# JiehongLin/SAM-6D

Measured on NVIDIA H100. Metric: poses/sec, higher is better.
Workload: dtype bf16

## Files before the change

include/sam6d_b200.h:

```cpp
#ifndef SAM6D_B200_H
#define SAM6D_B200_H

#ifdef __cplusplus
extern "C" {
#endif


int sam6d_fps(const float* xyz, int b, int n, int m, float* temp, int* idx, void* stream);
int sam6d_fps_single_cta(const float* xyz, int b, int n, int m, float* temp, int* idx, void* stream);

int sam6d_gather_points(const float* points, const int* idx, int b, int c, int n, int m, float* out, void* stream);

int sam6d_gather_rows(const float* src, const int* idx, int b, int n, int m, int c, long long src_bstride, float* out,
                      void* stream);
int sam6d_gather_rows_bf16_f32(const void* src, const int* idx, int b, int n, int m, int c, long long src_bstride, float* out,
                               void* stream);

int sam6d_ball_query(const float* new_xyz, const float* xyz, int b, int n, int m, float radius, int nsample, int* idx,
                     int* cnt, void* stream);
int sam6d_ball_query_pair(const float* new_xyz, const float* xyz, int b, int n, int m, float radius_a, int nsample_a,
                          float radius_b, int nsample_b, int* idx_a, int* idx_b, int* cnt_a, int* cnt_b, void* stream);

int sam6d_group_points(const float* points, const int* idx, int b, int c, int n, int np, int ns, float* out, void* stream);

// ... 132 lines not shown
int sam6d_linattn_apply(const float* Qf, long long q_rpb, long long q_bs, long long q_ld, const float* KV, const float* KS,
                        int B, int H, float* X, long long x_bs, long long x_ld, void* stream);
int sam6d_linattn_kv_pack(const float* Kf, long long k_ld, long long k_bs, const float* V, long long v_ld, long long v_bs, int B,
                          int J, void* blob, float* KS, void* stream);
int sam6d_linattn_tc(const void* Q, long long q_ld, long long q_bs, const void* blob, const float* KS,
                     const float* softplus_scale, int B, int rpb, void* X, long long x_ld, long long x_bs, void* stream);

int sam6d_coarse_assign(const float* A, int B, int S, float* W, float* w1, void* stream);
int sam6d_coarse_sample(const float* W, int B, int L, const float* rand, int nr, int* idx, void* stream);
int sam6d_coarse_hypotheses(const int* idx, const float* pts1, const float* pts2, int B, int n, int n1, float* Rt,
                            float* resid, void* stream);
int sam6d_topk_smallest(const float* v, int B, int n, int k, int* out, void* stream);
int sam6d_coarse_select(const float* Rt, const int* top, int B, int n1, int n2, const float* pts1, const float* w1, int n,
                        const float* model, int nm, float* scores, float* R, float* t, void* stream);
int sam6d_coarse_pick_distinct(const float* Rt, const int* top, const float* scores, int B, int n1, int n2, int K, float cos_thr,
                               float d2_min, float* R_out, float* t_out, float* score_out, unsigned char* valid, int* count,
                               void* stream);
int sam6d_coarse_pick_distinct_sym(const float* Rt, const int* top, const float* scores, int B, int n1, int n2, int K, float cos_thr,
                                   float d2_min, const float* symR, const float* symt, int S, const int* sym_range, int max_count,
                                   const float* radius, float* R_out, float* t_out, float* score_out, unsigned char* valid,
                                   int* count, void* stream);


int sam6d_pe_mlp_max(const float* pts, const int* idx, const int* cnt, int B, int N, int ns, const float* W1,
                     const float* B1, const float* W2, const float* B2, const float* W3, const float* B3, float* out,
                     int out_ld, int out_off, void* stream);
int sam6d_pe_mlp_max_tc(const float* pts, const int* idx, int B, int N, int ns, const float* W1, const float* B1,
                        const void* W2_bf16, const float* B2, const void* W3_bf16, const float* B3, void* out, int out_is_bf16,
                        int out_ld, int out_off, void* stream);
int sam6d_fine_assign(const float* A, int B, int S, int ld, float shift, const float* pts2, float* rsum, float* csum, float* cpart,
                      int* cpi, int* lab1, int* lab2, float* wts, float* pred, void* stream);
int sam6d_fine_pass_tc(const void* Fa, const void* Fb, int B, int S, float alpha, float shift, int mode, const float* row_f,
                       const float* col_f, int ld_f, const float* q4, float* out_inv, int* lab, float* wts, float* pred, void* stream);
int sam6d_fine_masked_points(const int* lab2, const float* pts2, int B, int S, int ld, float* q4, void* stream);
int sam6d_weighted_procrustes(const float* src, const float* ref, const float* wts, int B, int N, float weight_thresh,
                              float eps, float* R, float* t, void* stream);
int sam6d_pose_score(const float* pts1, const int* lab1, int B, int N, const float* R, const float* t, const float* model,
                     int nm, float dis_thres, const float* radius, float* score, float* t_scaled, void* stream);

int sam6d_bilinear_gather(const void* up, int up_is_bf16, const long long* choose, int B, int K, int G, int sub, int C, int H, int W,
                          float* out, void* stream);

int sam6d_attn_relpos(const float* qkv, long long tok_ld, int nW, int Hs, int Ws, int nH, int head_dim, const float* rel_h,
                      const float* rel_w, float scale, void* out, int out_is_bf16, long long out_ld, void* stream);

int sam6d_attn_global_tc(const void* qkv, long long ld, const void* Vt, long long vt_ld, const void* rel_blob, int B, int H, int grid,
                         float scale, void* out, int out_is_bf16, long long out_ld, void* stream);
int sam6d_attn_global_tc_ex(const void* qkv, long long ld, const void* Vt, long long vt_ld, const void* rel_blob, int B, int H, int grid,
                            int head_dim, float scale, void* out, int out_is_bf16, long long out_ld, void* stream);

int sam6d_icp_refine(const float* R, const float* t, const float* pts, int B, int N, const float* samples, const float* normals,
                     int O, int M, const int* obj, const float* radius, int iters, float* R_out, float* t_out, int* inliers,
                     float* rms, int* iters_run, int* corr, double* sums, void* stream);
int sam6d_icp_max_samples(void);

int sam6d_track_points(const float* rdepth, const unsigned short* depth, int O, int H, int W, float depth_scale, float fx, float fy,
                       float cx, float cy, const float* centre, const float* radius, int margin, int N, unsigned char* hmask,
                       unsigned char* cand, int* rows, float* pts, int* count, int* index, void* stream);
int sam6d_track_points_scene(const float* rdepth, const unsigned short* depth, int L, int H, int W, float depth_scale, float fx,
                             float fy, float cx, float cy, const float* centre, const float* radius, int margin, int N,
                             unsigned char* hmask, unsigned char* dmask, unsigned char* cand, int* rows, float* pts, int* count,
                             int* index, void* stream);

int sam6d_pose_verify(const float* rdepth, const float* depth, const unsigned char* mask, const int* mrow, const float* tau, int P,
                      int M, int H, int W, float rscale, int* counts, void* stream);

// ... 50 lines not shown
```

sam6d_b200/_lib.py:

```python
import ctypes
import os
import re

import torch

_Tensor = torch.Tensor

_HERE = os.path.dirname(os.path.abspath(__file__))
HEADER = os.path.join(os.path.dirname(_HERE), "include", "sam6d_b200.h")
LIB_PATH = os.path.join(_HERE, "libsam6d_b200.so")

_CTYPES = {
    "int": ctypes.c_int,
    "long long": ctypes.c_longlong,
    "float": ctypes.c_float,
    "double": ctypes.c_double,
}


def parse_header(path: str = HEADER):
    text = open(path).read()
    text = re.sub(r"/\*.*?\*/", "", text, flags=re.S)
    protos = {}
    for m in re.finditer(r"(const char\*|int)\s+(sam6d_\w+)\s*\(([^)]*)\)\s*;", text):
# ... 8 lines not shown
                typ, nm = a.rsplit(" ", 1)
                argl.append((_CTYPES[typ.strip()], nm))
        protos[name] = (ctypes.c_char_p if ret != "int" else ctypes.c_int, argl)
    return protos


class Sam6dError(RuntimeError):
    pass


_lib = None
_protos = None
_fns = {}


def lib():
    global _lib, _protos
    if _lib is None:
        if not os.path.exists(LIB_PATH):
            raise Sam6dError(
                f"{LIB_PATH} not found: build it with `python -m sam6d_b200.build` "
                "(or __graft_entry__.build()); sam6d_b200 has no CPU or eager fallback")
        _lib = ctypes.CDLL(LIB_PATH)
        _protos = parse_header()
        for name, (ret, args) in _protos.items():
            fn = getattr(_lib, name)
            fn.restype = ret
            fn.argtypes = [t for t, _ in args]
            _fns[name] = (fn, len(args) - 1 if args and args[-1][1] == "stream" else -1)
    return _lib


_launches = 0
_MULTI = {"sam6d_fine_assign": 6, "sam6d_coarse_select": 2, "sam6d_geo_embed_tc": 2, "sam6d_render_meshes": 4, "sam6d_yolo_masks": 2,
          "sam6d_mask_rle_count": 2, "sam6d_template_score_agg": 2, "sam6d_template_score": 2,
          "sam6d_pbr_reference_crops": 2, "sam6d_track_points": 4,
          "sam6d_track_points_scene": 5, "sam6d_symmetry_agreement": 2}
_timed = {}


def launch_count() -> int:
    return _launches


def add_launches(n: int):
    global _launches
    _launches += int(n)


def time_kernel(name: str, enable: bool = True):
    if enable:
        _timed[name] = []
    else:
        _timed.pop(name, None)


def timed_events(name: str):
    return _timed.get(name, [])


def call(name: str, *args):
    global _launches
    if _lib is None:
        lib()
    fn, n_before_stream = _fns[name]
    args = [(a.data_ptr() if a.is_cuda else _not_device(name, a)) if isinstance(a, _Tensor) else a for a in args]
    if len(args) == n_before_stream:
# ... 25 lines not shown
```

sam6d_b200/csrc/coarse.cu:

```cuda
#include "common.cuh"
#include "svd3.cuh"

namespace {

constexpr int ASSIGN_THREADS = 1024;
__global__ void __launch_bounds__(ASSIGN_THREADS) coarse_assign_kernel(const float* __restrict__ A, int S, float* __restrict__ W,
                                                            float* __restrict__ w1out) {
  extern __shared__ float sm[];
  float* a = sm;
  float* rmax = a + S * S;
  float* rsum = rmax + S;
  float* cmax = rsum + S;
  float* csum = cmax + S;
  int* lab1 = (int*)(csum + S);
  int* lab2 = lab1 + S;
  const int b = blockIdx.x, tid = threadIdx.x, lane = tid & 31, warp = tid >> 5;
  const float* Ab = A + (size_t)b * S * S;
  for (int e = tid; e < S * S; e += ASSIGN_THREADS) a[e] = Ab[e];
  __syncthreads();
  for (int i = warp; i < S; i += ASSIGN_THREADS / 32) {
    float m = -INFINITY;
    for (int j = lane; j < S; j += 32) m = fmaxf(m, a[i * S + j]);
    m = warp_max(m);
    float s = 0.f;
// ... 11 lines not shown
  __syncthreads();
  for (int e = tid; e < S * S; e += ASSIGN_THREADS) {
    int i = e / S, j = e - i * S;
    float v = a[e];
    a[e] = (expf(v - rmax[i]) / rsum[i]) * (expf(v - cmax[j]) / csum[j]);
  }
  __syncthreads();
  for (int i = warp; i < S; i += ASSIGN_THREADS / 32) {
    float bv = -INFINITY; int bi = 0x7fffffff;
    for (int j = lane; j < S; j += 32) argmax_first(bv, bi, a[i * S + j], j);
    warp_argmax_first(bv, bi);
    if (lane == 0) lab1[i] = bi;
  }
  for (int j = tid; j < S; j += ASSIGN_THREADS) {
    float bv = -INFINITY; int bi = 0;
    for (int i = 0; i < S; ++i) { float v = a[i * S + j]; if (v > bv) { bv = v; bi = i; } }
    lab2[j] = bi;
  }
  __syncthreads();
  const int n = S - 1;
  float* Wb = W + (size_t)b * n * n;
  for (int e = tid; e < n * n; e += ASSIGN_THREADS) {
    int i = e / n, j = e - i * n;
    float v = a[(i + 1) * S + (j + 1)];
    v = v * (lab1[i + 1] > 0 ? 1.f : 0.f) * (lab2[j + 1] > 0 ? 1.f : 0.f);
    Wb[e] = v * sqrtf(v);
  }
  for (int i = tid; i < n; i += ASSIGN_THREADS) w1out[(size_t)b * n + i] = lab1[i + 1] > 0 ? 1.f : 0.f;
}

__global__ void __launch_bounds__(1024) coarse_sample_kernel(const float* __restrict__ W, int L, const float* __restrict__ rand,
                                                             int nr, int* __restrict__ idx_out) {
  extern __shared__ float cdf[];
  __shared__ double part[1024];
  const int b = blockIdx.x, tid = threadIdx.x;
  const float* Wb = W + (size_t)b * L;
  const int per = (L + 1023) / 1024;
  const int beg = min(tid * per, L), end = min(beg + per, L);
  double s = 0.0;
  for (int i = beg; i < end; ++i) s += (double)Wb[i];
  part[tid] = s;
  __syncthreads();
  for (int o = 1; o < 1024; o <<= 1) {
    double v = (tid >= o) ? part[tid - o] : 0.0;
    __syncthreads();
    part[tid] += v;
    __syncthreads();
  }
  double run = (tid == 0) ? 0.0 : part[tid - 1];
  for (int i = beg; i < end; ++i) { run += (double)Wb[i]; cdf[i] = (float)run; }
  __syncthreads();
  const float denom = cdf[L - 1] + 1e-8f;
  __syncthreads();
  for (int i = tid; i < L; i += 1024) cdf[i] = cdf[i] / denom;
  __syncthreads();
  for (int r = tid; r < nr; r += 1024) {
    float v = rand[(size_t)b * nr + r];
    int lo = 0, hi = L;
    while (lo < hi) {
      int mid = (lo + hi) >> 1;
      if (cdf[mid] < v) lo = mid + 1; else hi = mid;
    }
    idx_out[(size_t)b * nr + r] = lo;
  }
}

__global__ void __launch_bounds__(128) coarse_hyp_kernel(const int* __restrict__ idx, const float* __restrict__ pts1,
                                                         const float* __restrict__ pts2, int n, int n1, float* __restrict__ Rt,
                                                         float* __restrict__ resid) {
  const int b = blockIdx.y;
  const int hpt = blockIdx.x * blockDim.x + threadIdx.x;
  if (hpt >= n1) return;
  const int* id = idx + ((size_t)b * n1 + hpt) * 3;
  float p1[3][3], p2[3][3];
  int i1s[3], i2s[3];
#pragma unroll
  for (int k = 0; k < 3; ++k) {
    int v = id[k];
    int i1 = min(v / n, n - 1), i2 = min(v % n, n - 1);
    i1s[k] = i1; i2s[k] = i2;
    const float* a = pts1 + ((size_t)b * n + i1) * 3;
    const float* c = pts2 + ((size_t)b * n + i2) * 3;
#pragma unroll
// ... 24 lines not shown
  if (rank0) {
#pragma unroll
    for (int i = 0; i < 3; ++i)
#pragma unroll
      for (int j = 0; j < 3; ++j) Rd[i][j] = (i == j) ? 1.0 : 0.0;
  } else {
    procrustes_rotation(H, Rd, rank1);
  }
  float R[3][3], t[3];
#pragma unroll
  for (int i = 0; i < 3; ++i)
#pragma unroll
    for (int j = 0; j < 3; ++j) R[i][j] = (float)Rd[i][j];
#pragma unroll
  for (int i = 0; i < 3; ++i) t[i] = cr[i] - (R[i][0] * cs[0] + R[i][1] * cs[1] + R[i][2] * cs[2]);
  float rs = 0.f;
#pragma unroll
  for (int k = 0; k < 3; ++k) {
    float x = p1[k][0] - t[0], y = p1[k][1] - t[1], z = p1[k][2] - t[2];
    float ex = x * R[0][0] + y * R[1][0] + z * R[2][0] - p2[k][0];
    float ey = x * R[0][1] + y * R[1][1] + z * R[2][1] - p2[k][1];
    float ez = x * R[0][2] + y * R[1][2] + z * R[2][2] - p2[k][2];
    rs += sqrtf(ex * ex + ey * ey + ez * ez);
  }
  float* o = Rt + ((size_t)b * n1 + hpt) * 12;
#pragma unroll
  for (int i = 0; i < 3; ++i)
#pragma unroll
    for (int j = 0; j < 3; ++j) o[i * 3 + j] = R[i][j];
  o[9] = t[0]; o[10] = t[1]; o[11] = t[2];
  resid[(size_t)b * n1 + hpt] = rs / 3.f;
}

__global__ void __launch_bounds__(1024) topk_smallest_kernel(const float* __restrict__ v, int n, int npow2, int k,
                                                             int* __restrict__ out) {
  extern __shared__ unsigned long long keys[];
  const int b = blockIdx.x, tid = threadIdx.x;
  for (int i = tid; i < npow2; i += 1024) {
    unsigned long long key = ~0ull;
    if (i < n) {
      float f = v[(size_t)b * n + i];
      unsigned u = __float_as_uint(f);
      u = (u & 0x80000000u) ? ~u : (u | 0x80000000u);
      key = ((unsigned long long)u << 32) | (unsigned)i;
    }
    keys[i] = key;
  }
  __syncthreads();
  for (int size = 2; size <= npow2; size <<= 1) {
    for (int stride = size >> 1; stride > 0; stride >>= 1) {
      for (int i = tid; i < npow2 / 2; i += 1024) {
        int lo = 2 * i - (i & (stride - 1));
        int hi = lo + stride;
        bool asc = ((lo & size) == 0);
        unsigned long long a = keys[lo], c = keys[hi];
        if ((a > c) == asc) { keys[lo] = c; keys[hi] = a; }
      }
      __syncthreads();
    }
  }
  for (int i = tid; i < k; i += 1024) out[(size_t)b * k + i] = (int)(keys[i] & 0xffffffffu);
}

constexpr int SEL_PP = 4, SEL_THREADS = 224;
__device__ __forceinline__ float min3f(float a, float b, float c) { return fminf(fminf(a, b), c); }
__global__ void __launch_bounds__(SEL_THREADS) coarse_select_kernel(const float* __restrict__ Rt, const int* __restrict__ top, int n1,
                                                                    int n2, const float* __restrict__ pts1, const float* __restrict__ w1,
                                                                    int n, const float* __restrict__ model, int nm,
                                                                    float* __restrict__ scores) {
  extern __shared__ float4 smq[];
  __shared__ float red[2 * SEL_PP][SEL_THREADS / 32];
  __shared__ float rts[SEL_PP][12];
  const int pose0 = blockIdx.x * SEL_PP, b = blockIdx.y, tid = threadIdx.x;
  for (int i = tid; i < nm; i += SEL_THREADS) {
    const float* q = model + ((size_t)b * nm + i) * 3;
    const float x = q[0], y = q[1], z = q[2];
    smq[i] = make_float4(x, y, z, x * x + y * y + z * z);
  }
  if (tid < SEL_PP * 12) {
    const int pp = tid / 12, e = tid - pp * 12;
    const int pose = min(pose0 + pp, n2 - 1);
    rts[pp][e] = Rt[((size_t)b * n1 + top[(size_t)b * n2 + pose]) * 12 + e];
  }
  __syncthreads();
  float num = 0.f, den[SEL_PP];
#pragma unroll
  for (int pp = 0; pp < SEL_PP; ++pp) den[pp] = 0.f;
  for (int i = tid; i < n; i += SEL_THREADS) {
    const float* p = pts1 + ((size_t)b * n + i) * 3;
    const float px = p[0], py = p[1], pz = p[2];
    float ax[SEL_PP], ay[SEL_PP], az[SEL_PP], x2[SEL_PP], best[SEL_PP];
#pragma unroll
    for (int pp = 0; pp < SEL_PP; ++pp) {
      const float* R = rts[pp];
// ... 209 lines not shown
  if (B == 0) return 0;
  size_t smem = ((size_t)S * S + 6 * S) * sizeof(float);
  S6_REQUIRE(smem <= 220 * 1024);
  S6_CHECK(cudaFuncSetAttribute(coarse_assign_kernel, cudaFuncAttributeMaxDynamicSharedMemorySize, (int)smem));
  coarse_assign_kernel<<<B, ASSIGN_THREADS, smem, s6_stream(stream)>>>(A, S, W, w1);
  S6_LAUNCH_CHECK();
  return 0;
}

S6_API int sam6d_coarse_sample(const float* W, int B, int L, const float* rand, int nr, int* idx, void* stream) {
  S6_REQUIRE(W && rand && idx && B >= 0 && L > 0 && nr >= 0);
  if (B == 0 || nr == 0) return 0;
  size_t smem = (size_t)L * sizeof(float);
  S6_REQUIRE(smem <= 200 * 1024);
  S6_CHECK(cudaFuncSetAttribute(coarse_sample_kernel, cudaFuncAttributeMaxDynamicSharedMemorySize, (int)smem));
  coarse_sample_kernel<<<B, 1024, smem, s6_stream(stream)>>>(W, L, rand, nr, idx);
  S6_LAUNCH_CHECK();
  return 0;
}

S6_API int sam6d_coarse_hypotheses(const int* idx, const float* pts1, const float* pts2, int B, int n, int n1, float* Rt,
                                   float* resid, void* stream) {
  S6_REQUIRE(idx && pts1 && pts2 && Rt && resid && B >= 0 && n > 0 && n1 >= 0);
  if (B == 0 || n1 == 0) return 0;
  dim3 grid(s6_cdiv(n1, 128), B);
  coarse_hyp_kernel<<<grid, 128, 0, s6_stream(stream)>>>(idx, pts1, pts2, n, n1, Rt, resid);
  S6_LAUNCH_CHECK();
  return 0;
}

S6_API int sam6d_topk_smallest(const float* v, int B, int n, int k, int* out, void* stream) {
  S6_REQUIRE(v && out && B >= 0 && n > 0 && k > 0 && k <= n);
  if (B == 0) return 0;
  int npow2 = 2;
  while (npow2 < n) npow2 <<= 1;
  size_t smem = (size_t)npow2 * sizeof(unsigned long long);
  S6_REQUIRE(smem <= 200 * 1024);
  S6_CHECK(cudaFuncSetAttribute(topk_smallest_kernel, cudaFuncAttributeMaxDynamicSharedMemorySize, (int)smem));
  topk_smallest_kernel<<<B, 1024, smem, s6_stream(stream)>>>(v, n, npow2, k, out);
  S6_LAUNCH_CHECK();
  return 0;
}

S6_API int sam6d_coarse_select(const float* Rt, const int* top, int B, int n1, int n2, const float* pts1, const float* w1, int n,
                               const float* model, int nm, float* scores, float* R, float* t, void* stream) {
  S6_REQUIRE(Rt && top && pts1 && w1 && model && scores && R && t && B >= 0 && n > 0 && nm > 0 && n2 > 0);
  if (B == 0) return 0;
  size_t smem = (size_t)nm * 4 * sizeof(float);
  S6_REQUIRE(smem <= 200 * 1024);
  S6_CHECK(cudaFuncSetAttribute(coarse_select_kernel, cudaFuncAttributeMaxDynamicSharedMemorySize, (int)smem));
  dim3 grid(s6_cdiv(n2, SEL_PP), B);
  coarse_select_kernel<<<grid, SEL_THREADS, smem, s6_stream(stream)>>>(Rt, top, n1, n2, pts1, w1, n, model, nm, scores);
  S6_LAUNCH_CHECK();
  coarse_pick_kernel<<<B, 32, 0, s6_stream(stream)>>>(scores, top, Rt, n1, n2, R, t);
  S6_LAUNCH_CHECK();
  return 0;
}

S6_API int sam6d_coarse_pick_distinct(const float* Rt, const int* top, const float* scores, int B, int n1, int n2, int K, float cos_thr,
                                      float d2_min, float* R_out, float* t_out, float* score_out, unsigned char* valid, int* count,
                                      void* stream) {
  S6_REQUIRE(B >= 0 && n1 > 0 && n2 > 0 && n2 <= PICK_MAX_N2 && K >= 1 && K <= n2);
  S6_REQUIRE(isfinite(cos_thr) && isfinite(d2_min));
  S6_REQUIRE(Rt && top && scores && R_out && t_out && score_out && valid && count);
  if (B == 0) return 0;
  const size_t smem = (size_t)n2 * 13 * sizeof(float) + n2;
  S6_CHECK(cudaFuncSetAttribute(coarse_pick_distinct_kernel, cudaFuncAttributeMaxDynamicSharedMemorySize, (int)smem));
  coarse_pick_distinct_kernel<<<B, PICK_THREADS, smem, s6_stream(stream)>>>(Rt, top, scores, n1, n2, K, cos_thr, d2_min, R_out, t_out,
                                                                          score_out, valid, count);
  S6_LAUNCH_CHECK();
  return 0;
}
// ... 19 lines not shown
```

sam6d_b200/csrc/fine_tc.cu:

```cuda
#include "common.cuh"
#include "tc.cuh"

namespace {

constexpr int BM = 128, BN = 256, BK = 64, KB = 4, STAGES = 4;
constexpr int A_KB = BM * BK * 2, B_KB = BN * BK * 2;
constexpr int CONSUMERS = 256, NUM_THREADS = CONSUMERS + 128;
constexpr int SMEM_BYTES = KB * A_KB + STAGES * B_KB + 1024;
constexpr float LOG2E = 1.4426950408889634f;

struct FArgs {
  int B, S, mode, ld_f;
  float a2, s2;
  const float* row_f;
  const float* col_f;
  const float4* q4;
  float* out_inv;
  int* lab;
  float* wts; float* pred;
};

__device__ __forceinline__ float ex2(float x) {
  float y;
  asm("ex2.approx.ftz.f32 %0, %1;" : "=f"(y) : "f"(x));
  return y;
}

template <int MODE>
__global__ void __launch_bounds__(NUM_THREADS, 1) fine_pass_kernel(const __grid_constant__ CUtensorMap tmA, const __grid_constant__ CUtensorMap tmB, FArgs g) {
  extern __shared__ __align__(1024) uint8_t smem_raw[];
  uint8_t* smem = reinterpret_cast<uint8_t*>((reinterpret_cast<uintptr_t>(smem_raw) + 1023) & ~(uintptr_t)1023);
  uint8_t* a_res = smem;
  uint8_t* ring = smem + KB * A_KB;
  __shared__ __align__(8) uint64_t a_full, a_empty, full_bar[STAGES], empty_bar[STAGES];
  __shared__ float sc[2][BN];
  __shared__ __align__(16) float4 sq[2][BN];

  const int tid = threadIdx.x, warp = tid >> 5, lane = tid & 31;
  const int m_tiles = (g.S + BM - 1) / BM, n_tiles = (g.S + BN - 1) / BN;
  const int items = g.B * m_tiles;

  if (tid == 0) {
    tc::mbar_init(&a_full, 1); tc::mbar_init(&a_empty, CONSUMERS / 32);
    for (int s = 0; s < STAGES; ++s) { tc::mbar_init(&full_bar[s], 1); tc::mbar_init(&empty_bar[s], CONSUMERS / 32); }
    tc::mbar_fence_init();
    tc::tma_prefetch_desc(&tmA);
    tc::tma_prefetch_desc(&tmB);
  }
  __syncthreads();

  if (warp >= CONSUMERS / 32) {
    tc::producer_regs();
    if (tid == CONSUMERS) {
      long long gk = 0;
      int it = 0;
      for (int item = blockIdx.x; item < items; item += gridDim.x, ++it) {
        const int b = item / m_tiles, mt = item - b * m_tiles;
        tc::mbar_wait(&a_empty, (uint32_t)((it & 1) ^ 1));
        tc::mbar_arrive_expect_tx(&a_full, KB * A_KB);
        for (int kb = 0; kb < KB; ++kb) tc::tma_load_2d(&tmA, &a_full, a_res + kb * A_KB, kb * BK, b * g.S + mt * BM);
        for (int nt = 0; nt < n_tiles; ++nt)
          for (int kb = 0; kb < KB; ++kb, ++gk) {
            const int s = (int)(gk % STAGES);
            tc::mbar_wait(&empty_bar[s], (uint32_t)(((gk / STAGES) & 1) ^ 1));
            tc::mbar_arrive_expect_tx(&full_bar[s], B_KB);
            tc::tma_load_2d(&tmB, &full_bar[s], ring + s * B_KB, kb * BK, b * g.S + nt * BN);
          }
      }
    }
    return;
  }
  tc::consumer_regs();
  const int wg = warp >> 2, w = warp & 3;
  const uint32_t a_addr = tc::smem_u32(a_res) + wg * (64 * 128);
  long long gk = 0, tcount = 0;
  int it = 0;
  for (int item = blockIdx.x; item < items; item += gridDim.x, ++it) {
    const int b = item / m_tiles, mt = item - b * m_tiles;
    float rf[2] = {0.f, 0.f};
#pragma unroll
    for (int hr = 0; hr < 2; ++hr) {
      const int i = mt * BM + wg * 64 + tc::frag_row(2 * hr, w, lane);
      if (MODE != 0 && i < g.S) rf[hr] = g.row_f[(size_t)b * g.ld_f + i];
    }
    const float* cf = (MODE != 0) ? g.col_f + (size_t)b * g.ld_f : nullptr;
    const float4* q4 = (MODE == 2) ? g.q4 + (size_t)b * g.ld_f : nullptr;
    float sum[2] = {0.f, 0.f}, bv[2] = {-INFINITY, -INFINITY}, ws[2] = {0.f, 0.f}, px[2] = {0.f, 0.f}, py[2] = {0.f, 0.f}, pz[2] = {0.f, 0.f};
    int bi[2] = {0x7fffffff, 0x7fffffff};
    tc::mbar_wait(&a_full, (uint32_t)(it & 1));
    for (int nt = 0; nt < n_tiles; ++nt, ++tcount) {
      const int buf = (int)(tcount & 1);
      if (MODE != 0) {
        const int j = nt * BN + tid;
        sc[buf][tid] = (j < g.S) ? cf[j] : 0.f;
        if (MODE == 2) sq[buf][tid] = (j < g.S) ? q4[j] : make_float4(0.f, 0.f, 0.f, 0.f);
        tc::named_bar(1, CONSUMERS);
      }
      float acc[BN / 2];
      int prev = -1;
      for (int kb = 0; kb < KB; ++kb, ++gk) {
        const int s = (int)(gk % STAGES);
        tc::mbar_wait(&full_bar[s], (uint32_t)((gk / STAGES) & 1));
        const uint32_t b_addr = tc::smem_u32(ring + s * B_KB);
        tc::wg_fence();
#pragma unroll
        for (int k = 0; k < BK / 16; ++k)
          tc::wgmma_bf16<BN>(acc, tc::wg_desc(a_addr + kb * A_KB + k * 32), tc::wg_desc(b_addr + k * 32), (kb | k) ? 1u : 0u);
        tc::wg_commit();
        if (prev >= 0) {
          tc::wg_wait<1>();
          if (lane == 0) tc::mbar_arrive(&empty_bar[prev]);
        }
        prev = s;
      }
      tc::wg_wait<0>();
      if (lane == 0) tc::mbar_arrive(&empty_bar[prev]);
      if (nt == n_tiles - 1 && lane == 0) tc::mbar_arrive(&a_empty);
#pragma unroll
      for (int e = 0; e < BN / 2; ++e) {
        const int hr = (e >> 1) & 1, cl = tc::frag_col(e, lane), j = nt * BN + cl;
        const float ev = (j < g.S) ? ex2(fmaf(acc[e], g.a2, -g.s2)) : 0.f;
        if (MODE == 0) {
          sum[hr] += ev;
        } else {
          const float p = (ev * rf[hr]) * (ev * sc[buf][cl]);
          if (p > bv[hr]) { bv[hr] = p; bi[hr] = j; }
          if (MODE == 2) {
            const float4 q = sq[buf][cl];
            const float pm = p * q.w;
            ws[hr] += pm; px[hr] = fmaf(pm, q.x, px[hr]); py[hr] = fmaf(pm, q.y, py[hr]); pz[hr] = fmaf(pm, q.z, pz[hr]);
          }
        }
      }
    }
#pragma unroll
    for (int hr = 0; hr < 2; ++hr) {
      const int i = mt * BM + wg * 64 + tc::frag_row(2 * hr, w, lane);
      if (MODE == 0) {
        const float t = tc::quad_sum(sum[hr]);
        if ((lane & 3) == 0 && i < g.S) g.out_inv[(size_t)b * g.ld_f + i] = 1.f / t;
      } else {
#pragma unroll
        for (int o = 1; o <= 2; o <<= 1) {
          const float ov = __shfl_xor_sync(0xffffffffu, bv[hr], o);
          const int oi = __shfl_xor_sync(0xffffffffu, bi[hr], o);
          if (ov > bv[hr] || (ov == bv[hr] && oi < bi[hr])) { bv[hr] = ov; bi[hr] = oi; }
        }
        float ww = 0.f, qx = 0.f, qy = 0.f, qz = 0.f;
        if (MODE == 2) { ww = tc::quad_sum(ws[hr]); qx = tc::quad_sum(px[hr]); qy = tc::quad_sum(py[hr]); qz = tc::quad_sum(pz[hr]); }
        if ((lane & 3) == 0 && i < g.S) {
          int lb = bi[hr];
          if (lb == 0x7fffffff) lb = 0;
          g.lab[(size_t)b * g.S + i] = lb;
          if (MODE == 2 && i >= 1) {
            if (lb == 0) { ww = 0.f; qx = 0.f; qy = 0.f; qz = 0.f; }
            const size_t o = (size_t)b * (g.S - 1) + (i - 1);
            const float d = ww + 1e-6f;
            g.wts[o] = ww;
            g.pred[o * 3 + 0] = qx / d; g.pred[o * 3 + 1] = qy / d; g.pred[o * 3 + 2] = qz / d;
          }
        }
      }
    }
  }
}

__global__ void fine_masked_points_kernel(const int* __restrict__ lab2, const float* __restrict__ pts2, int S, int ld, float4* __restrict__ q4) {
  const int b = blockIdx.y, j = blockIdx.x * blockDim.x + threadIdx.x;
  if (j >= ld) return;
  float4 q = make_float4(0.f, 0.f, 0.f, 0.f);
  if (j >= 1 && j < S && lab2[(size_t)b * S + j] > 0) {
    const float* p = pts2 + ((size_t)b * (S - 1) + (j - 1)) * 3;
    q = make_float4(p[0], p[1], p[2], 1.f);
  }
  q4[(size_t)b * ld + j] = q;
}

}

S6_API int sam6d_fine_pass_tc(const void* Fa, const void* Fb, int B, int S, float alpha, float shift, int mode, const float* row_f,
                              const float* col_f, int ld_f, const float* q4, float* out_inv, int* lab, float* wts, float* pred,
                              void* stream) {
  S6_REQUIRE(Fa && Fb && B >= 0 && S >= 2 && mode >= 0 && mode <= 2 && ld_f >= S);
  S6_REQUIRE(((reinterpret_cast<uintptr_t>(Fa) | reinterpret_cast<uintptr_t>(Fb)) & 15) == 0 && (long long)B * S < 2000000000LL);
  if (mode == 0) S6_REQUIRE(out_inv != nullptr);
  if (mode >= 1) S6_REQUIRE(row_f && col_f && lab);
  if (mode == 2) S6_REQUIRE(q4 && wts && pred && (reinterpret_cast<uintptr_t>(q4) & 15) == 0);
  if (B == 0) return 0;
  CUtensorMap tmA, tmB;
  int rc = tc::make_map_2d(&tmA, Fa, (long long)B * S, 256, 256, 64, BM);
  if (rc) return rc;
  rc = tc::make_map_2d(&tmB, Fb, (long long)B * S, 256, 256, 64, BN);
  if (rc) return rc;
  int grid;
  S6_CHECK(s6_persistent_grid(B * s6_cdiv(S, BM), 1, &grid));
  FArgs g{B, S, mode, ld_f, alpha * LOG2E, shift * LOG2E, row_f, col_f, reinterpret_cast<const float4*>(q4), out_inv, lab, wts, pred};
  cudaStream_t st = s6_stream(stream);
#define FINE_LAUNCH(M)                                                                                              \
  do {                                                                                                              \
    S6_CHECK(cudaFuncSetAttribute(fine_pass_kernel<M>, cudaFuncAttributeMaxDynamicSharedMemorySize, SMEM_BYTES));   \
    fine_pass_kernel<M><<<grid, NUM_THREADS, SMEM_BYTES, st>>>(tmA, tmB, g);                                        \
  } while (0)
  if (mode == 0) FINE_LAUNCH(0); else if (mode == 1) FINE_LAUNCH(1); else FINE_LAUNCH(2);
#undef FINE_LAUNCH
  S6_LAUNCH_CHECK();
  return 0;
}

S6_API int sam6d_fine_masked_points(const int* lab2, const float* pts2, int B, int S, int ld, float* q4, void* stream) {
  S6_REQUIRE(lab2 && pts2 && q4 && B >= 0 && S >= 2 && ld >= S && (reinterpret_cast<uintptr_t>(q4) & 15) == 0);
  if (B == 0) return 0;
  dim3 grid(s6_cdiv(ld, 256), B);
  fine_masked_points_kernel<<<grid, 256, 0, s6_stream(stream)>>>(lab2, pts2, S, ld, reinterpret_cast<float4*>(q4));
  S6_LAUNCH_CHECK();
  return 0;
}
```

sam6d_b200/ops.py:

```python
from typing import Optional, Tuple

import numpy as np
import torch

from . import _lib

Tensor = torch.Tensor


def _check(t: Tensor, dtype, name: str, ndim: Optional[int] = None):
    if not isinstance(t, torch.Tensor):
        raise RuntimeError(f"{name} must be a torch.Tensor")
    if not t.is_cuda:
        raise RuntimeError(f"{name} must be a CUDA tensor (CPU not supported)")
    if t.dtype != dtype:
        raise RuntimeError(f"{name} must be {dtype}, got {t.dtype}")
    if not t.is_contiguous():
        raise RuntimeError(f"{name} must be contiguous")
    if ndim is not None and t.dim() != ndim:
        raise RuntimeError(f"{name} must have {ndim} dims, got {t.dim()}")


def _rows(t: Tensor) -> Tuple[int, int, int]:
    if t.dim() not in (2, 3) or t.stride(-1) != 1:
# ... 691 lines not shown
    if A.stride(2) != 1 or A.stride(0) != S * A.stride(1) or A.stride(1) % 4 or A.data_ptr() % 16:
        ld = (S + 3) // 4 * 4
        store = torch.empty(B, S, ld, dtype=torch.float32, device=A.device)
        store[:, :, :S] = A
        A = store[:, :, :S]
    ld = A.stride(1)
    dev = A.device
    tiles = (S + 31) // 32
    if tiles < 4:
        raise RuntimeError("fine_assign: S >= 97 required")
    rsum = torch.empty(B, ld, dtype=torch.float32, device=dev)
    csum = torch.empty(B, ld, dtype=torch.float32, device=dev)
    cpart = torch.empty(B, tiles, ld, dtype=torch.float32, device=dev)
    cpi = torch.empty(B, tiles, ld, dtype=torch.int32, device=dev)
    lab1 = torch.zeros(B, S, dtype=torch.int32, device=dev)
    lab2 = torch.zeros(B, S, dtype=torch.int32, device=dev)
    wts = torch.empty(B, S - 1, dtype=torch.float32, device=dev)
    pred = torch.empty(B, S - 1, 3, dtype=torch.float32, device=dev)
    _lib.call("sam6d_fine_assign", A, B, S, int(ld), shift, pts2, rsum, csum, cpart, cpi, lab1, lab2, wts, pred)
    return lab1, lab2, wts, pred


def fine_assign_tc(f1n: Tensor, f2n: Tensor, pts2: Tensor, alpha: float):
    _check(f1n, torch.bfloat16, "f1n", 3)
    _check(f2n, torch.bfloat16, "f2n", 3)
    _check(pts2, torch.float32, "pts2", 3)
    B, S, C = f1n.shape
    if C != 256 or f2n.shape != f1n.shape or pts2.shape[1] != S - 1:
        raise RuntimeError("fine_assign_tc: (B,S,256) tokens and (B,S-1,3) points expected")
    dev = f1n.device
    ld = (S + 3) // 4 * 4
    rinv = torch.empty(B, ld, dtype=torch.float32, device=dev)
    cinv = torch.empty(B, ld, dtype=torch.float32, device=dev)
    q4 = torch.empty(B, ld, 4, dtype=torch.float32, device=dev)
    lab1 = torch.zeros(B, S, dtype=torch.int32, device=dev)
    lab2 = torch.zeros(B, S, dtype=torch.int32, device=dev)
    wts = torch.empty(B, S - 1, dtype=torch.float32, device=dev)
    pred = torch.empty(B, S - 1, 3, dtype=torch.float32, device=dev)
    _lib.call("sam6d_fine_pass_tc", f1n, f2n, B, S, alpha, alpha, 0, None, None, ld, None, rinv, None, None, None)
    _lib.call("sam6d_fine_pass_tc", f2n, f1n, B, S, alpha, alpha, 0, None, None, ld, None, cinv, None, None, None)
    _lib.call("sam6d_fine_pass_tc", f2n, f1n, B, S, alpha, alpha, 1, cinv, rinv, ld, None, None, lab2, None, None)
    _lib.call("sam6d_fine_masked_points", lab2, pts2, B, S, ld, q4)
    _lib.call("sam6d_fine_pass_tc", f1n, f2n, B, S, alpha, alpha, 2, rinv, cinv, ld, q4, None, lab1, wts, pred)
    return lab1, lab2, wts, pred


def weighted_procrustes(src: Tensor, ref: Tensor, wts: Tensor, weight_thresh: float = 0.0, eps: float = 1e-5):
    _check(src, torch.float32, "src", 3)
    _check(ref, torch.float32, "ref", 3)
    _check(wts, torch.float32, "weights", 2)
    B, N, _ = src.shape
    R = torch.empty(B, 3, 3, dtype=torch.float32, device=src.device)
    t = torch.empty(B, 3, dtype=torch.float32, device=src.device)
    _lib.call("sam6d_weighted_procrustes", src, ref, wts, B, N, weight_thresh, eps, R, t)
    return R, t


def pose_score(pts1: Tensor, lab1: Tensor, R: Tensor, t: Tensor, model: Tensor, radius: Tensor, dis_thres: float = 0.15):
    _check(pts1, torch.float32, "pts1", 3)
    _check(lab1, torch.int32, "lab1", 2)
    B, N, _ = pts1.shape
    score = torch.empty(B, dtype=torch.float32, device=pts1.device)
    ts = torch.empty(B, 3, dtype=torch.float32, device=pts1.device)
    _lib.call("sam6d_pose_score", pts1, lab1, B, N, R, t, model, model.shape[1], dis_thres, radius, score, ts)
    return score, ts


def icp_max_samples() -> int:
    m = _lib.lib().sam6d_icp_max_samples()
    if m < 0:
        raise _lib.Sam6dError(f"sam6d_icp_max_samples: CUDA error {-m}")
    return m

# ... 260 lines not shown
```

Baseline: 2632.

## Fuse fine row/column softmax sums, radix-select topk, warp-scan coarse sampling

Computes the fine-matching column sums as per-tile partials inside the row-sum pass and reduces them in a small kernel, replacing a second full tensor-core GEMM pass with the transposed operands. Also replaces the bitonic-sort top-k with a byte-wise radix select followed by ranking of the k selected keys, and changes the coarse sampling prefix sum to a warp-shuffle scan over weights staged in shared memory. These cut duplicated GEMM work, sort work, and block-wide barriers, at the cost of a partials buffer, extra shuffles and a named barrier in the epilogue, and an O(k^2) ranking step.

```diff
diff --git a/include/sam6d_b200.h b/include/sam6d_b200.h
--- a/include/sam6d_b200.h
+++ b/include/sam6d_b200.h
@@ -188,6 +188,8 @@
                       int* cpi, int* lab1, int* lab2, float* wts, float* pred, void* stream);
 int sam6d_fine_pass_tc(const void* Fa, const void* Fb, int B, int S, float alpha, float shift, int mode, const float* row_f,
                        const float* col_f, int ld_f, const float* q4, float* out_inv, int* lab, float* wts, float* pred, void* stream);
+int sam6d_fine_sums_tc(const void* F1, const void* F2, int B, int S, float alpha, float shift, int ld, float* rinv, float* cinv,
+                       float* colpart, void* stream);
 int sam6d_fine_masked_points(const int* lab2, const float* pts2, int B, int S, int ld, float* q4, void* stream);
 int sam6d_weighted_procrustes(const float* src, const float* ref, const float* wts, int B, int N, float weight_thresh,
                               float eps, float* R, float* t, void* stream);
diff --git a/sam6d_b200/_lib.py b/sam6d_b200/_lib.py
--- a/sam6d_b200/_lib.py
+++ b/sam6d_b200/_lib.py
@@ -64,7 +64,7 @@
 
 
 _launches = 0
-_MULTI = {"sam6d_fine_assign": 6, "sam6d_coarse_select": 2, "sam6d_geo_embed_tc": 2, "sam6d_render_meshes": 4, "sam6d_yolo_masks": 2,
+_MULTI = {"sam6d_fine_assign": 6, "sam6d_fine_sums_tc": 2, "sam6d_coarse_select": 2, "sam6d_geo_embed_tc": 2, "sam6d_render_meshes": 4, "sam6d_yolo_masks": 2,
           "sam6d_mask_rle_count": 2, "sam6d_template_score_agg": 2, "sam6d_template_score": 2,
           "sam6d_pbr_reference_crops": 2, "sam6d_track_points": 4,
           "sam6d_track_points_scene": 5, "sam6d_symmetry_agreement": 2}
diff --git a/sam6d_b200/csrc/coarse.cu b/sam6d_b200/csrc/coarse.cu
--- a/sam6d_b200/csrc/coarse.cu
+++ b/sam6d_b200/csrc/coarse.cu
@@ -67,23 +67,35 @@
 __global__ void __launch_bounds__(1024) coarse_sample_kernel(const float* __restrict__ W, int L, const float* __restrict__ rand,
                                                              int nr, int* __restrict__ idx_out) {
   extern __shared__ float cdf[];
-  __shared__ double part[1024];
-  const int b = blockIdx.x, tid = threadIdx.x;
+  __shared__ double wtot[32];
+  const int b = blockIdx.x, tid = threadIdx.x, lane = tid & 31, warp = tid >> 5;
   const float* Wb = W + (size_t)b * L;
+  for (int i = tid; i < L; i += 1024) cdf[i] = Wb[i];
+  __syncthreads();
   const int per = (L + 1023) / 1024;
   const int beg = min(tid * per, L), end = min(beg + per, L);
   double s = 0.0;
-  for (int i = beg; i < end; ++i) s += (double)Wb[i];
-  part[tid] = s;
-  __syncthreads();
-  for (int o = 1; o < 1024; o <<= 1) {
-    double v = (tid >= o) ? part[tid - o] : 0.0;
-    __syncthreads();
-    part[tid] += v;
-    __syncthreads();
-  }
-  double run = (tid == 0) ? 0.0 : part[tid - 1];
-  for (int i = beg; i < end; ++i) { run += (double)Wb[i]; cdf[i] = (float)run; }
+  for (int i = beg; i < end; ++i) s += (double)cdf[i];
+  double incl = s;
+#pragma unroll
+  for (int o = 1; o < 32; o <<= 1) {
+    const double y = __shfl_up_sync(0xffffffffu, incl, o);
+    if (lane >= o) incl += y;
+  }
+  if (lane == 31) wtot[warp] = incl;
+  __syncthreads();
+  if (warp == 0) {
+    double t = wtot[lane];
+#pragma unroll
+    for (int o = 1; o < 32; o <<= 1) {
+      const double y = __shfl_up_sync(0xffffffffu, t, o);
+      if (lane >= o) t += y;
+    }
+    wtot[lane] = t;
+  }
+  __syncthreads();
+  double run = (warp ? wtot[warp - 1] : 0.0) + (incl - s);
+  for (int i = beg; i < end; ++i) { run += (double)cdf[i]; cdf[i] = (float)run; }
   __syncthreads();
   const float denom = cdf[L - 1] + 1e-8f;
   __syncthreads();
@@ -174,34 +186,64 @@
   resid[(size_t)b * n1 + hpt] = rs / 3.f;
 }
 
-__global__ void __launch_bounds__(1024) topk_smallest_kernel(const float* __restrict__ v, int n, int npow2, int k,
-                                                             int* __restrict__ out) {
-  extern __shared__ unsigned long long keys[];
-  const int b = blockIdx.x, tid = threadIdx.x;
-  for (int i = tid; i < npow2; i += 1024) {
-    unsigned long long key = ~0ull;
-    if (i < n) {
-      float f = v[(size_t)b * n + i];
-      unsigned u = __float_as_uint(f);
-      u = (u & 0x80000000u) ? ~u : (u | 0x80000000u);
-      key = ((unsigned long long)u << 32) | (unsigned)i;
-    }
-    keys[i] = key;
-  }
-  __syncthreads();
-  for (int size = 2; size <= npow2; size <<= 1) {
-    for (int stride = size >> 1; stride > 0; stride >>= 1) {
-      for (int i = tid; i < npow2 / 2; i += 1024) {
-        int lo = 2 * i - (i & (stride - 1));
-        int hi = lo + stride;
-        bool asc = ((lo & size) == 0);
-        unsigned long long a = keys[lo], c = keys[hi];
-        if ((a > c) == asc) { keys[lo] = c; keys[hi] = a; }
+constexpr int TOPK_THREADS = 1024, TOPK_MAX_N = 16384;
+__device__ __forceinline__ unsigned long long topk_key(const unsigned* u, int i) { return ((unsigned long long)u[i] << 32) | (unsigned)i; }
+__global__ void __launch_bounds__(TOPK_THREADS) topk_smallest_kernel(const float* __restrict__ v, int n, int k, int* __restrict__ out) {
+  extern __shared__ unsigned long long sel[];
+  unsigned* u = reinterpret_cast<unsigned*>(sel + k);
+  __shared__ int hist[256];
+  __shared__ int s_digit, s_rem, s_count, s_n;
+  const int b = blockIdx.x, tid = threadIdx.x, lane = tid & 31;
+  for (int i = tid; i < n; i += TOPK_THREADS) {
+    const unsigned x = __float_as_uint(v[(size_t)b * n + i]);
+    u[i] = (x & 0x80000000u) ? ~x : (x | 0x80000000u);
+  }
+  unsigned long long prefix = 0;
+  int rem = k, shift = 56;
+  for (;; shift -= 8) {
+    if (tid < 256) hist[tid] = 0;
+    __syncthreads();
+    for (int i = tid; i < n; i += TOPK_THREADS) {
+      const unsigned long long key = topk_key(u, i);
+      if (shift == 56 || (key >> (shift + 8)) == (prefix >> (shift + 8))) atomicAdd(&hist[(int)(key >> shift) & 255], 1);
+    }
+    __syncthreads();
+    if (tid < 32) {
+      int c[8], run = 0;
+#pragma unroll
+      for (int d = 0; d < 8; ++d) { run += hist[lane * 8 + d]; c[d] = run; }
+      int incl = run;
+#pragma unroll
+      for (int o = 1; o < 32; o <<= 1) {
+        const int y = __shfl_up_sync(0xffffffffu, incl, o);
+        if (lane >= o) incl += y;
       }
-      __syncthreads();
-    }
-  }
-  for (int i = tid; i < k; i += 1024) out[(size_t)b * k + i] = (int)(keys[i] & 0xffffffffu);
+      const int before = incl - run;
+      if (before < rem && rem <= incl) {
+        int d = 0;
+        while (before + c[d] < rem) ++d;
+        const int below = before + (d ? c[d - 1] : 0);
+        s_digit = lane * 8 + d; s_rem = rem - below; s_count = c[d] - (d ? c[d - 1] : 0);
+      }
+    }
+    if (tid == 0) s_n = 0;
+    __syncthreads();
+    prefix |= (unsigned long long)s_digit << shift;
+    rem = s_rem;
+    if (s_count == rem) break;
+    __syncthreads();
+  }
+  for (int i = tid; i < n; i += TOPK_THREADS) {
+    const unsigned long long key = topk_key(u, i);
+    if ((key >> shift) <= (prefix >> shift)) sel[atomicAdd(&s_n, 1)] = key;
+  }
+  __syncthreads();
+  for (int j = tid; j < k; j += TOPK_THREADS) {
+    const unsigned long long key = sel[j];
+    int r = 0;
+    for (int x = 0; x < k; ++x) r += sel[x] < key;
+    out[(size_t)b * k + r] = (int)(key & 0xffffffffu);
+  }
 }
 
 constexpr int SEL_PP = 4, SEL_THREADS = 224;
@@ -477,12 +519,10 @@
 S6_API int sam6d_topk_smallest(const float* v, int B, int n, int k, int* out, void* stream) {
   S6_REQUIRE(v && out && B >= 0 && n > 0 && k > 0 && k <= n);
   if (B == 0) return 0;
-  int npow2 = 2;
-  while (npow2 < n) npow2 <<= 1;
-  size_t smem = (size_t)npow2 * sizeof(unsigned long long);
-  S6_REQUIRE(smem <= 200 * 1024);
+  S6_REQUIRE(n <= TOPK_MAX_N);
+  const size_t smem = (size_t)k * sizeof(unsigned long long) + (size_t)n * sizeof(unsigned);
   S6_CHECK(cudaFuncSetAttribute(topk_smallest_kernel, cudaFuncAttributeMaxDynamicSharedMemorySize, (int)smem));
-  topk_smallest_kernel<<<B, 1024, smem, s6_stream(stream)>>>(v, n, npow2, k, out);
+  topk_smallest_kernel<<<B, TOPK_THREADS, smem, s6_stream(stream)>>>(v, n, k, out);
   S6_LAUNCH_CHECK();
   return 0;
 }
diff --git a/sam6d_b200/csrc/fine_tc.cu b/sam6d_b200/csrc/fine_tc.cu
--- a/sam6d_b200/csrc/fine_tc.cu
+++ b/sam6d_b200/csrc/fine_tc.cu
@@ -16,6 +16,7 @@
   const float* col_f;
   const float4* q4;
   float* out_inv;
+  float* colpart;
   int* lab;
   float* wts; float* pred;
 };
@@ -24,6 +25,35 @@
   float y;
   asm("ex2.approx.ftz.f32 %0, %1;" : "=f"(y) : "f"(x));
   return y;
+}
+
+__device__ __forceinline__ void col_partials(const float (&v)[32], float (&cp)[CONSUMERS / 32][BN], float* __restrict__ out, int j0,
+                                             int ld, int warp, int lane, int tid) {
+  const bool hi4 = lane & 16, hi3 = lane & 8, hi2 = lane & 4;
+  float v2[16], v3[8];
+#pragma unroll
+  for (int m = 0; m < 8; ++m)
+#pragma unroll
+    for (int p = 0; p < 2; ++p) {
+      const float ev = v[4 * m + p], od = v[4 * m + 2 + p];
+      v2[2 * m + p] = (hi3 ? od : ev) + __shfl_xor_sync(0xffffffffu, hi3 ? ev : od, 8);
+    }
+#pragma unroll
+  for (int n = 0; n < 4; ++n)
+#pragma unroll
+    for (int p = 0; p < 2; ++p) {
+      const float ev = v2[4 * n + p], od = v2[4 * n + 2 + p];
+      v3[2 * n + p] = (hi2 ? od : ev) + __shfl_xor_sync(0xffffffffu, hi2 ? ev : od, 4);
+    }
+#pragma unroll
+  for (int n = 0; n < 4; ++n)
+#pragma unroll
+    for (int p = 0; p < 2; ++p) cp[warp][8 * (8 * n + 4 * hi2 + 2 * hi3 + hi4) + 2 * (lane & 3) + p] = v3[2 * n + p];
+  tc::named_bar(2, CONSUMERS);
+  float t = cp[0][tid];
+#pragma unroll
+  for (int w = 1; w < CONSUMERS / 32; ++w) t += cp[w][tid];
+  if (j0 + tid < ld) out[j0 + tid] = t;
 }
 
 template <int MODE>
@@ -35,6 +65,7 @@
   __shared__ __align__(8) uint64_t a_full, a_empty, full_bar[STAGES], empty_bar[STAGES];
   __shared__ float sc[2][BN];
   __shared__ __align__(16) float4 sq[2][BN];
+  __shared__ float cp[MODE == 0 ? 2 : 1][CONSUMERS / 32][MODE == 0 ? BN : 1];
 
   const int tid = threadIdx.x, warp = tid >> 5, lane = tid & 31;
   const int m_tiles = (g.S + BM - 1) / BM, n_tiles = (g.S + BN - 1) / BN;
@@ -87,6 +118,8 @@
     const float4* q4 = (MODE == 2) ? g.q4 + (size_t)b * g.ld_f : nullptr;
     float sum[2] = {0.f, 0.f}, bv[2] = {-INFINITY, -INFINITY}, ws[2] = {0.f, 0.f}, px[2] = {0.f, 0.f}, py[2] = {0.f, 0.f}, pz[2] = {0.f, 0.f};
     int bi[2] = {0x7fffffff, 0x7fffffff};
+    const bool colp = MODE == 0 && g.colpart != nullptr;
+    const bool row0 = mt * BM + wg * 64 + tc::frag_row(0, w, lane) < g.S, row1 = mt * BM + wg * 64 + tc::frag_row(2, w, lane) < g.S;
     tc::mbar_wait(&a_full, (uint32_t)(it & 1));
     for (int nt = 0; nt < n_tiles; ++nt, ++tcount) {
       const int buf = (int)(tcount & 1);
@@ -116,21 +149,34 @@
       tc::wg_wait<0>();
       if (lane == 0) tc::mbar_arrive(&empty_bar[prev]);
       if (nt == n_tiles - 1 && lane == 0) tc::mbar_arrive(&a_empty);
+      if constexpr (MODE == 0) {
+        float v[32], keep[2], cs[2];
+#pragma unroll
+        for (int e = 0; e < BN / 2; ++e) {
+          const int hr = (e >> 1) & 1, p = e & 1, c = e >> 2, j = nt * BN + tc::frag_col(e, lane);
+          const float ev = (j < g.S) ? ex2(fmaf(acc[e], g.a2, -g.s2)) : 0.f;
+          sum[hr] += ev;
+          const float m = (hr ? row1 : row0) ? ev : 0.f;
+          cs[p] = hr ? cs[p] + m : m;
+          if (colp && hr == 1) {
+            if (c & 1) v[2 * (c >> 1) + p] = ((lane & 16) ? cs[p] : keep[p]) + __shfl_xor_sync(0xffffffffu, (lane & 16) ? keep[p] : cs[p], 16);
+            else keep[p] = cs[p];
+          }
+        }
+        if (colp) col_partials(v, cp[buf], g.colpart + ((size_t)b * m_tiles + mt) * g.ld_f, nt * BN, g.ld_f, warp, lane, tid);
+      } else {
 #pragma unroll
       for (int e = 0; e < BN / 2; ++e) {
         const int hr = (e >> 1) & 1, cl = tc::frag_col(e, lane), j = nt * BN + cl;
         const float ev = (j < g.S) ? ex2(fmaf(acc[e], g.a2, -g.s2)) : 0.f;
-        if (MODE == 0) {
-          sum[hr] += ev;
-        } else {
-          const float p = (ev * rf[hr]) * (ev * sc[buf][cl]);
-          if (p > bv[hr]) { bv[hr] = p; bi[hr] = j; }
-          if (MODE == 2) {
-            const float4 q = sq[buf][cl];
-            const float pm = p * q.w;
-            ws[hr] += pm; px[hr] = fmaf(pm, q.x, px[hr]); py[hr] = fmaf(pm, q.y, py[hr]); pz[hr] = fmaf(pm, q.z, pz[hr]);
-          }
-        }
+        const float p = (ev * rf[hr]) * (ev * sc[buf][cl]);
+        if (p > bv[hr]) { bv[hr] = p; bi[hr] = j; }
+        if (MODE == 2) {
+          const float4 q = sq[buf][cl];
+          const float pm = p * q.w;
+          ws[hr] += pm; px[hr] = fmaf(pm, q.x, px[hr]); py[hr] = fmaf(pm, q.y, py[hr]); pz[hr] = fmaf(pm, q.z, pz[hr]);
+        }
+      }
       }
     }
 #pragma unroll
@@ -176,6 +222,34 @@
   q4[(size_t)b * ld + j] = q;
 }
 
+__global__ void fine_col_inv_kernel(const float* __restrict__ colpart, int S, int ld, int m_tiles, float* __restrict__ cinv) {
+  const int b = blockIdx.y, j = blockIdx.x * blockDim.x + threadIdx.x;
+  if (j >= S) return;
+  const float* p = colpart + (size_t)b * m_tiles * ld + j;
+  float t = 0.f;
+  for (int mt = 0; mt < m_tiles; ++mt) t += p[(size_t)mt * ld];
+  cinv[(size_t)b * ld + j] = 1.f / t;
+}
+
+int launch_fine_pass(const void* Fa, const void* Fb, const FArgs& g, cudaStream_t st) {
+  CUtensorMap tmA, tmB;
+  int rc = tc::make_map_2d(&tmA, Fa, (long long)g.B * g.S, 256, 256, 64, BM);
+  if (rc) return rc;
+  rc = tc::make_map_2d(&tmB, Fb, (long long)g.B * g.S, 256, 256, 64, BN);
+  if (rc) return rc;
+  int grid;
+  S6_CHECK(s6_persistent_grid(g.B * s6_cdiv(g.S, BM), 1, &grid));
+#define FINE_LAUNCH(M)                                                                                              \
+  do {                                                                                                              \
+    S6_CHECK(cudaFuncSetAttribute(fine_pass_kernel<M>, cudaFuncAttributeMaxDynamicSharedMemorySize, SMEM_BYTES));   \
+    fine_pass_kernel<M><<<grid, NUM_THREADS, SMEM_BYTES, st>>>(tmA, tmB, g);                                        \
+  } while (0)
+  if (g.mode == 0) FINE_LAUNCH(0); else if (g.mode == 1) FINE_LAUNCH(1); else FINE_LAUNCH(2);
+#undef FINE_LAUNCH
+  S6_LAUNCH_CHECK();
+  return 0;
+}
+
 }
 
 S6_API int sam6d_fine_pass_tc(const void* Fa, const void* Fb, int B, int S, float alpha, float shift, int mode, const float* row_f,
@@ -187,22 +261,21 @@
   if (mode >= 1) S6_REQUIRE(row_f && col_f && lab);
   if (mode == 2) S6_REQUIRE(q4 && wts && pred && (reinterpret_cast<uintptr_t>(q4) & 15) == 0);
   if (B == 0) return 0;
-  CUtensorMap tmA, tmB;
-  int rc = tc::make_map_2d(&tmA, Fa, (long long)B * S, 256, 256, 64, BM);
+  FArgs g{B, S, mode, ld_f, alpha * LOG2E, shift * LOG2E, row_f, col_f, reinterpret_cast<const float4*>(q4), out_inv, nullptr, lab, wts, pred};
+  return launch_fine_pass(Fa, Fb, g, s6_stream(stream));
+}
+
+S6_API int sam6d_fine_sums_tc(const void* F1, const void* F2, int B, int S, float alpha, float shift, int ld, float* rinv, float* cinv,
+                              float* colpart, void* stream) {
+  S6_REQUIRE(F1 && F2 && rinv && cinv && colpart && B >= 0 && S >= 2 && ld >= S);
+  S6_REQUIRE(((reinterpret_cast<uintptr_t>(F1) | reinterpret_cast<uintptr_t>(F2)) & 15) == 0 && (long long)B * S < 2000000000LL);
+  if (B == 0) return 0;
+  FArgs g{B, S, 0, ld, alpha * LOG2E, shift * LOG2E, nullptr, nullptr, nullptr, rinv, colpart, nullptr, nullptr, nullptr};
+  cudaStream_t st = s6_stream(stream);
+  const int rc = launch_fine_pass(F1, F2, g, st);
   if (rc) return rc;
-  rc = tc::make_map_2d(&tmB, Fb, (long long)B * S, 256, 256, 64, BN);
-  if (rc) return rc;
-  int grid;
-  S6_CHECK(s6_persistent_grid(B * s6_cdiv(S, BM), 1, &grid));
-  FArgs g{B, S, mode, ld_f, alpha * LOG2E, shift * LOG2E, row_f, col_f, reinterpret_cast<const float4*>(q4), out_inv, lab, wts, pred};
-  cudaStream_t st = s6_stream(stream);
-#define FINE_LAUNCH(M)                                                                                              \
-  do {                                                                                                              \
-    S6_CHECK(cudaFuncSetAttribute(fine_pass_kernel<M>, cudaFuncAttributeMaxDynamicSharedMemorySize, SMEM_BYTES));   \
-    fine_pass_kernel<M><<<grid, NUM_THREADS, SMEM_BYTES, st>>>(tmA, tmB, g);                                        \
-  } while (0)
-  if (mode == 0) FINE_LAUNCH(0); else if (mode == 1) FINE_LAUNCH(1); else FINE_LAUNCH(2);
-#undef FINE_LAUNCH
+  dim3 grid(s6_cdiv(S, 256), B);
+  fine_col_inv_kernel<<<grid, 256, 0, st>>>(colpart, S, ld, s6_cdiv(S, BM), cinv);
   S6_LAUNCH_CHECK();
   return 0;
 }
diff --git a/sam6d_b200/ops.py b/sam6d_b200/ops.py
--- a/sam6d_b200/ops.py
+++ b/sam6d_b200/ops.py
@@ -747,13 +747,13 @@
     ld = (S + 3) // 4 * 4
     rinv = torch.empty(B, ld, dtype=torch.float32, device=dev)
     cinv = torch.empty(B, ld, dtype=torch.float32, device=dev)
+    colpart = torch.empty(B, (S + 127) // 128, ld, dtype=torch.float32, device=dev)
     q4 = torch.empty(B, ld, 4, dtype=torch.float32, device=dev)
     lab1 = torch.zeros(B, S, dtype=torch.int32, device=dev)
     lab2 = torch.zeros(B, S, dtype=torch.int32, device=dev)
     wts = torch.empty(B, S - 1, dtype=torch.float32, device=dev)
     pred = torch.empty(B, S - 1, 3, dtype=torch.float32, device=dev)
-    _lib.call("sam6d_fine_pass_tc", f1n, f2n, B, S, alpha, alpha, 0, None, None, ld, None, rinv, None, None, None)
-    _lib.call("sam6d_fine_pass_tc", f2n, f1n, B, S, alpha, alpha, 0, None, None, ld, None, cinv, None, None, None)
+    _lib.call("sam6d_fine_sums_tc", f1n, f2n, B, S, alpha, alpha, ld, rinv, cinv, colpart)
     _lib.call("sam6d_fine_pass_tc", f2n, f1n, B, S, alpha, alpha, 1, cinv, rinv, ld, None, None, lab2, None, None)
     _lib.call("sam6d_fine_masked_points", lab2, pts2, B, S, ld, q4)
     _lib.call("sam6d_fine_pass_tc", f1n, f2n, B, S, alpha, alpha, 2, rinv, cinv, ld, q4, None, lab1, wts, pred)
```

Result: faster. 2683, median of 6 (+1.9%).
